# ashawkey/nerf2mesh

Measured on NVIDIA H100. Metric: ray-samples/sec (train step), higher is better.
Workload: dtype fp16

## Files before the change

nerf2mesh_b200/csrc/fused.cu:

```cuda
#include "n2m_common.cuh"
#include "s0_geom.cuh"
#include "mlp_common.cuh"
#include "../../include/n2m_b200_fused.h"

namespace n2m {
namespace {

__device__ __forceinline__ void bar_mlp() { asm volatile("bar.sync 1, 128;" ::: "memory"); }
__device__ __forceinline__ void sync_mlp() {
    wg::fence_async_smem();
    bar_mlp();
}
__device__ __forceinline__ void mbar_arrive1(uint64_t* bar) {
    asm volatile("mbarrier.arrive.shared::cta.b64 _, [%0];" :: "r"(wg::smem_u32(bar)) : "memory");
}

constexpr uint32_t kFwdThreads = 384;
constexpr uint32_t FF_W = 0, FF_A0 = FF_W + W_BYTES, FF_A1 = FF_A0 + kTileBytes, FF_H = FF_A1 + kTileBytes, FF_S1 = FF_H + kTileBytes,
                   FF_AS2 = FF_S1 + 8192, FF_BYTES = FF_AS2 + 4096;

__device__ __forceinline__ void bar_group(uint32_t g) {
    if (g == 0) asm volatile("bar.sync 2, 128;" ::: "memory");
    else asm volatile("bar.sync 3, 128;" ::: "memory");
}

__global__ void __launch_bounds__(kFwdThreads, 2)
k_s0_fwd_fused(n2m_s0_params p, const float4* __restrict__ recs, const int32_t* __restrict__ counters, const float* __restrict__ rays_o,
               const float* __restrict__ rays_d, const TableEntry* __restrict__ table, const int32_t* __restrict__ offsets,
               const uint8_t* __restrict__ wpack, uint8_t* __restrict__ enc_tiles, float4* __restrict__ out, float* __restrict__ spec_sq_sum) {
    extern __shared__ __align__(128) uint8_t smem[];
    __shared__ uint64_t bar_full[2], bar_empty[2];
    __shared__ float red[4];
    const uint32_t tid = threadIdx.x, warp = tid >> 5;
    const PartRange pr = part_range(counters, 0, 1);
    const uint32_t t1 = (pr.hi + kTile - 1) / kTile;
    if (pr.hi == 0 || blockIdx.x >= t1) return;
    const uint32_t my_tiles = (t1 - blockIdx.x + gridDim.x - 1) / gridDim.x;

    if (tid == 0) {
        wg::mbar_init(&bar_full[0], 1); wg::mbar_init(&bar_full[1], 1);
        wg::mbar_init(&bar_empty[0], 1); wg::mbar_init(&bar_empty[1], 1);
        wg::mbar_init_fence();
    }
    for (uint32_t i = tid; i < W_BYTES / 16; i += kFwdThreads)
        reinterpret_cast<uint4*>(smem + FF_W)[i] = __ldg(reinterpret_cast<const uint4*>(wpack) + i);
    if (tid < 128) *reinterpret_cast<uint4*>(smem + FF_AS2 + kChunk + tid * 16) = make_uint4(0, 0, 0, 0);
    wg::fence_async_smem();
    __syncthreads();

    if (warp >= 4) {
        const uint32_t g = (warp - 4) >> 2, r = tid - 128 - g * 128;
        uint8_t* buf = smem + (g ? FF_A1 : FF_A0);
        uint32_t k = 0;
        for (uint32_t it = g; it < my_tiles; it += 2, ++k) {
            const uint32_t tile = blockIdx.x + it * gridDim.x;
            float feat[kTileCols];
            encode_fwd_features<false>(p, recs, rays_o, rays_d, table, offsets, pr, tile * kTile + r, feat);
            if (r == 0) {
                asm volatile("cp.async.bulk.wait_group.read 0;" ::: "memory");
                wg::mbar_wait(&bar_empty[g], (k & 1) ^ 1);
            }
            bar_group(g);
            store_tile_row(buf, r, feat);
            wg::fence_async_smem();
            bar_group(g);
            if (r == 0) {
                asm volatile("cp.async.bulk.global.shared::cta.bulk_group [%0], [%1], %2;"
                             :: "l"(enc_tiles + (size_t)tile * kTileBytes), "r"(wg::smem_u32(buf)), "r"(kTileBytes) : "memory");
                asm volatile("cp.async.bulk.commit_group;" ::: "memory");
                mbar_arrive1(&bar_full[g]);
            }
        }
        if (r == 0) asm volatile("cp.async.bulk.wait_group 0;" ::: "memory");
    } else {
        float spec_sq = 0.f;
        const uint32_t r = sample_row(tid);
        for (uint32_t it = 0; it < my_tiles; ++it) {
            const uint32_t tile = blockIdx.x + it * gridDim.x, g = it & 1;
            const uint8_t* sA = smem + (g ? FF_A1 : FF_A0);
            wg::mbar_wait(&bar_full[g], (it >> 1) & 1);
            float sp[3];
            const float4 o = mlp_fwd_tile(sA, smem + FF_W, smem + FF_H, smem + FF_S1, smem + FF_S1, smem + FF_AS2, p.shading_full != 0,
                                          tid, sp, sync_mlp);
            const uint32_t j = tile * kTile + r;
            if (j < pr.hi) {
                out[j] = o;
                spec_sq += sp[0] * sp[0] + sp[1] * sp[1] + sp[2] * sp[2];
            }
            sync_mlp();
            if (tid == 0) mbar_arrive1(&bar_empty[g]);
        }
#pragma unroll
        for (int o = 16; o > 0; o >>= 1) spec_sq += __shfl_xor_sync(0xffffffffu, spec_sq, o);
        if ((tid & 31) == 0) red[warp] = spec_sq;
        bar_mlp();
        if (tid == 0 && spec_sq_sum) atomicAdd(spec_sq_sum, red[0] + red[1] + red[2] + red[3]);
// ... 29 lines not shown
```

nerf2mesh_b200/csrc/s0_geom.cuh:

```cuda
#pragma once
#include "n2m_common.cuh"
#include "../../include/n2m_b200_fused.h"

namespace n2m {
namespace {

constexpr uint32_t kTile = 128;
constexpr uint32_t kTileCols = 64;
constexpr uint32_t kTileBytes = kTile * kTileCols * 2;
constexpr uint32_t kChunkBytes = kTile * 16;
constexpr uint32_t kColXyz = 0, kColDens = 3, kColColor = 19, kColDir = 51;
constexpr uint32_t kLevels = 16;

struct __align__(8) TableEntry { float d; __half2 c; };

struct Sample {
    float x, y, z;
    float u, v, w;
    float dx, dy, dz;
};

__device__ __forceinline__ Sample sample_of(const float4 rec, const float* __restrict__ rays_o,
                                            const float* __restrict__ rays_d, const n2m_s0_params& p) {
    Sample s;
// ... 65 lines not shown
        zs[0] = z0 * mz;            zs[1] = zs[0] + mz;
    }
    const float wx[2] = {1 - fx, fx}, wy[2] = {1 - fy, fy}, wz[2] = {1 - fz, fz};
    const bool pow2 = (g.rows & (g.rows - 1)) == 0;
#pragma unroll
    for (int k = 0; k < 8; ++k) {
        const int ix = k & 1, iy = (k >> 1) & 1, iz = (k >> 2) & 1;
        const uint32_t raw = hashed ? (xs[ix] ^ ys[iy] ^ zs[iz]) : (xs[ix] + ys[iy] + zs[iz]);
        c.row[k] = wrap_row(raw, g.rows, pow2);
        c.w[k] = wx[ix] * wy[iy] * wz[iz];
    }
    if (left) {
        uint32_t lx, ly, lz;
        if (hashed) {
            lx = (x0 - 1u) ^ ys[0] ^ zs[0];
            ly = xs[0] ^ (ys[0] - 2654435761u) ^ zs[0];
            lz = xs[0] ^ ys[0] ^ (zs[0] - 805459861u);
        } else {
            lx = xs[0] - mx + ys[0] + zs[0];
            ly = xs[0] + ys[0] - my + zs[0];
            lz = xs[0] + ys[0] + zs[0] - mz;
        }
        left[0] = wrap_row(lx, g.rows, pow2);
        left[1] = wrap_row(ly, g.rows, pow2);
        left[2] = wrap_row(lz, g.rows, pow2);
    }
}

__device__ __forceinline__ uint32_t pack2(float a, float b) {
    const __half2 h = __floats2half2_rn(a, b);
    return *reinterpret_cast<const uint32_t*>(&h);
}

template <bool POINTS>
__device__ __forceinline__ bool
encode_fwd_features(const n2m_s0_params& p, const float4* __restrict__ recs, const float* __restrict__ rays_o,
                    const float* __restrict__ rays_d, const TableEntry* __restrict__ table, const int32_t* __restrict__ offsets,
                    const PartRange pr, uint32_t j, float (&feat)[kTileCols]) {
#pragma unroll
    for (uint32_t i = 0; i < kTileCols; ++i) feat[i] = 0.f;
    Sample s;
    const bool own = j >= pr.lo && j < pr.hi;
    bool active = own;
    if (own) {
        if (POINTS) {
            s.x = rays_o[3 * j]; s.y = rays_o[3 * j + 1]; s.z = rays_o[3 * j + 2];
            s.u = __fmul_rn(__fadd_rn(s.x, p.grid_bound), p.inv_2gb);
            s.v = __fmul_rn(__fadd_rn(s.y, p.grid_bound), p.inv_2gb);
            s.w = __fmul_rn(__fadd_rn(s.z, p.grid_bound), p.inv_2gb);
            s.dx = rays_d ? rays_d[3 * j] : 0.f; s.dy = rays_d ? rays_d[3 * j + 1] : 0.f; s.dz = rays_d ? rays_d[3 * j + 2] : 1.f;
        } else
        s = sample_of(recs[j], rays_o, rays_d, p);
        feat[kColXyz] = s.x; feat[kColXyz + 1] = s.y; feat[kColXyz + 2] = s.z;
        const float n2 = __fadd_rn(__fadd_rn(__fmul_rn(s.dx, s.dx), __fmul_rn(s.dy, s.dy)), __fmul_rn(s.dz, s.dz));
        const float nrm = __fsqrt_rn(fmaxf(n2, 1e-20f));
        feat[kColDir] = __fdiv_rn(s.dx, nrm); feat[kColDir + 1] = __fdiv_rn(s.dy, nrm); feat[kColDir + 2] = __fdiv_rn(s.dz, nrm);
        active = !((s.u < 0 || s.u > 1) || (s.v < 0 || s.v > 1) || (s.w < 0 || s.w > 1));
    } else {
        s.x = s.y = s.z = s.u = s.v = s.w = 0.5f; s.dx = s.dy = s.dz = 0.f;
    }
#pragma unroll
    for (uint32_t l = 0; l < kLevels; ++l) {
        const LevelGeom g = level_geom(offsets, l, p.S, p.base_res);
        Corners c; uint32_t base[3]; bool hashed;
        corners_of(g, s.u, s.v, s.w, c, base, hashed, nullptr);
        const TableEntry* tab = table + g.row0;
        if (active) {
            uint2 raw[8];
#pragma unroll
            for (int k = 0; k < 8; ++k) raw[k] = __ldg(reinterpret_cast<const uint2*>(tab + c.row[k]));
            float d = 0.f, c0 = 0.f, c1 = 0.f;
#pragma unroll
            for (int k = 0; k < 8; ++k) {
                const float2 cc = __half22float2(*reinterpret_cast<const __half2*>(&raw[k].y));
                d += c.w[k] * __uint_as_float(raw[k].x);
                c0 += c.w[k] * cc.x;
                c1 += c.w[k] * cc.y;
            }
            feat[kColDens + l] = d;
            feat[kColColor + 2 * l] = c0;
            feat[kColColor + 2 * l + 1] = c1;
        }
    }
    return own;
}

__device__ __forceinline__ float denc_col(const uint8_t* row, uint32_t col) {
    return __half2float(__ldg(reinterpret_cast<const __half*>(row + (col >> 3) * kChunkBytes + (col & 7) * 2)));
}

__device__ __forceinline__ void store_tile_row(uint8_t* img, uint32_t r, const float (&feat)[kTileCols]) {
    uint8_t* dst = img + r * 16;
#pragma unroll
    for (uint32_t ch = 0; ch < 8; ++ch) {
        uint4 q;
        q.x = pack2(feat[8 * ch + 0], feat[8 * ch + 1]);
        q.y = pack2(feat[8 * ch + 2], feat[8 * ch + 3]);
        q.z = pack2(feat[8 * ch + 4], feat[8 * ch + 5]);
        q.w = pack2(feat[8 * ch + 6], feat[8 * ch + 7]);
        *reinterpret_cast<uint4*>(dst + ch * kChunkBytes) = q;
    }
}

}
}
```

nerf2mesh_b200/csrc/stage0.cu:

```cuda
#include "march_core.cuh"
#include "s0_geom.cuh"
#include <cstdlib>
#include "../../include/n2m_b200_fused.h"

namespace n2m {
namespace {

using namespace march;

__global__ void __launch_bounds__(128)
k_s0_count(const float* __restrict__ rays_o, const float* __restrict__ rays_d, const float* __restrict__ aabb,
           const float* __restrict__ cam_nf, const uint8_t* __restrict__ bits, const float* __restrict__ noises,
           n2m_s0_params p, uint32_t N, int32_t* __restrict__ rays, float2* __restrict__ tbuf) {
    const uint32_t n = blockIdx.x * blockDim.x + threadIdx.x;
    if (n >= N) return;
    const MarchCfg c = make_cfg(p.bound, p.contract != 0, p.dt_gamma, p.max_steps, p.cascades, p.grid_size, bits);
    float near, far;
    near_far_aabb(rays_o + 3 * n, rays_d + 3 * n, aabb, p.min_near, near, far);
    if (cam_nf) {
        near = fmaxf(near, cam_nf[2 * n]);
        far = fminf(far, cam_nf[2 * n + 1]);
    }
    const float ox = rays_o[3 * n], oy = rays_o[3 * n + 1], oz = rays_o[3 * n + 2];
    const float dx = rays_d[3 * n], dy = rays_d[3 * n + 1], dz = rays_d[3 * n + 2];
// ... 134 lines not shown
        counters[3] = 0;
        counters[15] = 0;
        if (M > Mcap) counters[13] += 1;
        counters[14] = max(counters[14], (int32_t)M);
    }
    if (threadIdx.x <= kPartSlots) {
        const uint32_t e = threadIdx.x;
        const uint32_t first = part_first_ray(N, e);
        const uint32_t off = (e == kPartSlots || first >= N) ? M : (uint32_t)rays[2 * first];
        counters[4 + e] = (int32_t)min(min(off, M), Mcap);
    }
}

__global__ void __launch_bounds__(256)
k_s0_records(const int32_t* __restrict__ rays, const float2* __restrict__ tbuf, uint32_t N, uint32_t max_steps,
             uint32_t Mcap, float4* __restrict__ recs) {
    const uint32_t n = (blockIdx.x * blockDim.x + threadIdx.x) >> 5;
    const uint32_t lane = threadIdx.x & 31;
    if (n >= N) return;
    const uint32_t off = (uint32_t)rays[2 * n], cnt = (uint32_t)rays[2 * n + 1];
    const float2* slab = tbuf + (size_t)n * max_steps;
    for (uint32_t k = lane; k < cnt; k += 32) {
        const uint32_t j = off + k;
        if (j >= Mcap) break;
        const float2 td = slab[k];
        recs[j] = make_float4(td.x, td.y, td.x + td.y, __int_as_float((int)n));
    }
}

template <bool POINTS>
__device__ __forceinline__ void
encode_fwd_tile(const n2m_s0_params& p, const float4* __restrict__ recs,
                const float* __restrict__ rays_o, const float* __restrict__ rays_d,
                const TableEntry* __restrict__ table, const int32_t* __restrict__ offsets,
                uint8_t* __restrict__ enc_tiles, const PartRange pr, uint32_t nparts, uint32_t tile) {
    float feat[kTileCols];
    const bool own = encode_fwd_features<POINTS>(p, recs, rays_o, rays_d, table, offsets, pr, tile * kTile + threadIdx.x, feat);
    if (nparts > 1 && !own) return;
    store_tile_row(enc_tiles + (size_t)tile * kTileBytes, threadIdx.x, feat);
}

template <bool POINTS>
__global__ void __launch_bounds__(kTile, 6)
k_s0_encode_fwd(n2m_s0_params p, const float4* __restrict__ recs, const int32_t* __restrict__ counters,
                const float* __restrict__ rays_o, const float* __restrict__ rays_d,
                const TableEntry* __restrict__ table, const int32_t* __restrict__ offsets,
                uint8_t* __restrict__ enc_tiles, uint32_t part, uint32_t nparts) {
    const PartRange pr = part_range(counters, part, nparts);
    if (pr.hi <= pr.lo) return;
    const uint32_t t1 = (pr.hi + kTile - 1) / kTile;
#pragma unroll 1
    for (uint32_t tile = pr.lo / kTile + blockIdx.x; tile < t1; tile += gridDim.x)
        encode_fwd_tile<POINTS>(p, recs, rays_o, rays_d, table, offsets, enc_tiles, pr, nparts, tile);
}

__device__ __forceinline__ float tv_grad(const TableEntry* __restrict__ tab, const Corners& c, const uint32_t base[3],
                                         const uint32_t left[3], uint32_t res, float w) {
    const int right_corner[3] = {1, 2, 4};
    const float centre = __ldg(&tab[c.row[0]].d);
    float rv[3], lv[3];
#pragma unroll
    for (int d = 0; d < 3; ++d) {
        rv[d] = __ldg(&tab[c.row[right_corner[d]]].d);
        lv[d] = base[d] > 0 ? __ldg(&tab[left[d]].d) : 0.f;
    }
    float sum = 0.f, sq = 0.f;
#pragma unroll
    for (int d = 0; d < 3; ++d) {
        if (base[d] < res) { const float dv = centre - rv[d]; sum += dv; sq += dv * dv; }
        if (base[d] > 0) { const float dv = centre - lv[d]; sum += dv; sq += dv * dv; }
    }
    return w * sum * rsqrtf(sq + 1e-9f);
}

constexpr uint32_t kDenseGroupLevels = 5;
constexpr uint32_t kHashedGroupLevels = 1;
constexpr uint32_t kLevelGroups = 1 + (kLevels - kDenseGroupLevels + kHashedGroupLevels - 1) / kHashedGroupLevels;

__device__ __forceinline__ uint32_t group_first_level(uint32_t grp) {
    return grp == 0 ? 0u : min(kLevels, kDenseGroupLevels + (grp - 1) * kHashedGroupLevels);
}

__device__ __forceinline__ uint64_t l2_evict_last() {
    uint64_t pol;
    asm("createpolicy.fractional.L2::evict_last.b64 %0, 1.0;" : "=l"(pol));
    return pol;
}
__device__ __forceinline__ void red_add_v4(float4* dst, float a, float b, float c, uint64_t pol) {
    asm volatile("red.global.add.L2::cache_hint.v4.f32 [%0], {%1, %2, %3, %4}, %5;"
                 :: "l"(dst), "f"(a), "f"(b), "f"(c), "f"(0.f), "l"(pol) : "memory");
}

template <bool SCATTER, bool TV>
__device__ __forceinline__ void
encode_bwd_visit(const n2m_s0_params& p, const float4* __restrict__ recs,
                 const float* __restrict__ rays_o, const float* __restrict__ rays_d,
                 const uint8_t* __restrict__ denc_tiles, const TableEntry* __restrict__ table,
                 const int32_t* __restrict__ offsets, float4* __restrict__ gtable, float* __restrict__ loss_scale,
                 const PartRange pr, uint32_t tile, uint32_t l0, uint32_t l1, int32_t* tv_counts) {
    static_assert(SCATTER != TV, "a launch either scatters the feature gradients or evaluates TV");
    const uint32_t r = threadIdx.x;
    const uint32_t lane = r & 31;
    const uint32_t j = tile * kTile + r;
    Sample s;
    bool active = j >= pr.lo && j < pr.hi;
    if (active) {
        s = sample_of(recs[j], rays_o, rays_d, p);
        active = !((s.u < 0 || s.u > 1) || (s.v < 0 || s.v > 1) || (s.w < 0 || s.w > 1));
    } else {
        s.x = s.y = s.z = s.u = s.v = s.w = 0.5f; s.dx = s.dy = s.dz = 0.f;
    }

    const uint8_t* img = denc_tiles + (size_t)tile * kTileBytes + r * 16;
    bool bad = false;
    float tvw_lane = 0.f;
    if (TV) {
        const float mag = fmaxf(fabsf(s.x), fmaxf(fabsf(s.y), fabsf(s.z)));
        const bool outer = p.grid_bound > 1 && mag > 1;
        const float lam = outer ? p.lambda_tv * 10 : p.lambda_tv;
        tvw_lane = active ? lam / 6 * loss_scale[0] : 0.f;
        const bool mine = j >= pr.lo && j < pr.hi;
        const uint32_t m_out = __ballot_sync(0xffffffffu, mine && outer), m_in = __ballot_sync(0xffffffffu, mine && !outer);
        if (lane == 0 && l0 == 0) {
            if (m_in) atomicAdd(tv_counts + 3, (int)__popc(m_in));
            if (m_out) atomicAdd(tv_counts + 15, (int)__popc(m_out));
        }
    }
#pragma unroll 1
    for (uint32_t l = l0; l < l1; ++l) {
        const LevelGeom lg = level_geom(offsets, l, p.S, p.base_res);
        Corners c; uint32_t base[3]; bool hashed; uint32_t left[3];
        corners_of(lg, s.u, s.v, s.w, c, base, hashed, TV ? left : nullptr);
        float tvw = tvw_lane;
        float4* gt = gtable + lg.row0;
// ... 31 lines not shown
                }
            }
            const bool tail = lane == 31 || ((heads >> (lane + 1)) & 1u);
            issue = active && tail;
        }
        if (issue) {
            if (SCATTER) {
#pragma unroll
                const uint64_t pol = l2_evict_last();
#pragma unroll
                for (int k = 0; k < 8; ++k) red_add_v4(gt + c.row[k], vd[k], v0[k], v1[k], pol);
            }
            if (TV) atomicAdd(&gt[c.row[0]].x, tv_grad(table + lg.row0, c, base, left, lg.res, tvw));
        }
    }
    if (SCATTER && bad) loss_scale[3] = 1.f;
}

template <bool SCATTER, bool TV>
__global__ void __launch_bounds__(kTile)
k_s0_encode_bwd(n2m_s0_params p, const float4* __restrict__ recs, const int32_t* __restrict__ counters,
                const float* __restrict__ rays_o, const float* __restrict__ rays_d,
                const uint8_t* __restrict__ denc_tiles, const TableEntry* __restrict__ table,
                const int32_t* __restrict__ offsets, float4* __restrict__ gtable, float* __restrict__ loss_scale,
                uint32_t part, uint32_t nparts) {
    const PartRange pr = part_range(counters, part, nparts);
    if (pr.hi <= pr.lo) return;
    const uint32_t t0 = pr.lo / kTile, nt = (pr.hi + kTile - 1) / kTile - t0;
#pragma unroll 1
    for (uint32_t item = blockIdx.x; item < kLevelGroups * nt; item += gridDim.x) {
        const uint32_t grp = item / nt;
        encode_bwd_visit<SCATTER, TV>(p, recs, rays_o, rays_d, denc_tiles, table, offsets, gtable, loss_scale, pr, t0 + item % nt,
                                      group_first_level(grp), group_first_level(grp + 1), const_cast<int32_t*>(counters));
    }
}

__host__ __device__ __forceinline__ uint32_t mix32(uint32_t h) {
    h ^= h >> 16; h *= 0x85ebca6bu; h ^= h >> 13; h *= 0xc2b2ae35u; h ^= h >> 16;
    return h;
}
__host__ __device__ __forceinline__ float tv_random_coord(uint32_t seed, uint32_t idx, uint32_t axis) {
    return (float)(mix32(mix32(idx * 3u + axis) ^ (seed * 0x9e3779b9u)) >> 8) * (1.0f / 16777216.0f);
}

__global__ void __launch_bounds__(128)
k_s0_tv_random(n2m_s0_params p, const int32_t* __restrict__ counters, const TableEntry* __restrict__ table,
               const int32_t* __restrict__ offsets, float4* __restrict__ gtable, const float* __restrict__ loss_scale, uint32_t B,
               float* __restrict__ dump) {
    float lam = 0.f;
    if (p.grid_bound > 1) {
        if (counters[3] == 0) lam += p.lambda_tv;
        if (counters[15] == 0) lam += p.lambda_tv * 10;
    } else if (counters[3] + counters[15] == 0) lam = p.lambda_tv;
    if (dump) lam = p.lambda_tv;
    if (!(lam > 0.f)) return;
    const uint32_t i = blockIdx.x * blockDim.x + threadIdx.x;
    if (i >= B) return;
    const uint32_t seed = (uint32_t)loss_scale[2];
    const float u = tv_random_coord(seed, i, 0), v = tv_random_coord(seed, i, 1), w = tv_random_coord(seed, i, 2);
    if (dump) { dump[3 * i] = u; dump[3 * i + 1] = v; dump[3 * i + 2] = w; }
    const float tvw = lam / 6 * loss_scale[0];
#pragma unroll 1
    for (uint32_t l = 0; l < kLevels; ++l) {
        const LevelGeom lg = level_geom(offsets, l, p.S, p.base_res);
        Corners c; uint32_t base[3]; bool hashed; uint32_t left[3];
        corners_of(lg, u, v, w, c, base, hashed, left);
// ... 211 lines not shown
    cmaster[i] = c;
}

__global__ void __launch_bounds__(256)
k_s0_unpack_tables(const TableEntry* __restrict__ table, const float2* __restrict__ cmaster, uint32_t rows,
                   float* __restrict__ ed, float* __restrict__ ec) {
    const uint32_t i = blockIdx.x * blockDim.x + threadIdx.x;
    if (i >= rows) return;
    ed[i] = table[i].d;
    ec[2 * i] = cmaster[i].x; ec[2 * i + 1] = cmaster[i].y;
}

__global__ void __launch_bounds__(256)
k_s0_unpack_grads(const float4* __restrict__ gtable, uint32_t rows, const float* __restrict__ loss_scale,
                  float* __restrict__ gd, float* __restrict__ gc) {
    const uint32_t i = blockIdx.x * blockDim.x + threadIdx.x;
    if (i >= rows) return;
    const float inv = 1.0f / loss_scale[0];
    const float4 g = gtable[i];
    gd[i] = g.x * inv; gc[2 * i] = g.y * inv; gc[2 * i + 1] = g.z * inv;
}

}
}

using namespace n2m;

static bool g_serial_march = false;

static inline uint32_t part_grid(uint32_t Mcap, uint32_t nparts) {
    return nparts <= 1 ? Mcap / kTile : div_up(Mcap / kTile, nparts) + 1;
}

template <bool SCATTER, bool TV>
static uint32_t encode_bwd_grid(uint32_t Mcap, uint32_t nparts, uint32_t share = 1) {
    static int per_sm = 0;
    if (!per_sm) {
        cudaOccupancyMaxActiveBlocksPerMultiprocessor(&per_sm, k_s0_encode_bwd<SCATTER, TV>, kTile, 0);
        if (per_sm <= 0) per_sm = 1;
    }
    return min(max(1u, (uint32_t)(per_sm * num_sms()) / (nparts * share)), kLevelGroups * part_grid(Mcap, nparts));
}

constexpr uint32_t kTvDeviceShare = 2;

extern "C" {

int n2m_s0_set_serial_march(int on) { g_serial_march = on != 0; return 0; }
int n2m_s0_pack_tables(const float* emb_density, const float* emb_color, uint32_t rows, void* table, void* color_master,
                       n2m_stream_t stream) {
    N2M_REQUIRE(emb_density && emb_color && table && color_master, "s0_pack_tables", "null pointer");
    k_s0_pack_tables<<<div_up(rows, 256u), 256, 0, as_stream(stream)>>>(emb_density, emb_color, rows,
                                                                         static_cast<TableEntry*>(table), static_cast<float2*>(color_master));
    return check_launch("s0_pack_tables");
}

int n2m_s0_unpack_tables(const void* table, const void* color_master, uint32_t rows, float* emb_density, float* emb_color,
                         n2m_stream_t stream) {
    N2M_REQUIRE(emb_density && emb_color && table && color_master, "s0_unpack_tables", "null pointer");
    k_s0_unpack_tables<<<div_up(rows, 256u), 256, 0, as_stream(stream)>>>(static_cast<const TableEntry*>(table),
                                                                           static_cast<const float2*>(color_master), rows, emb_density, emb_color);
    return check_launch("s0_unpack_tables");
}

int n2m_s0_unpack_grads(const void* gtable, uint32_t rows, const float* loss_scale, float* g_density, float* g_color,
                        n2m_stream_t stream) {
    N2M_REQUIRE(gtable && loss_scale && g_density && g_color, "s0_unpack_grads", "null pointer");
    k_s0_unpack_grads<<<div_up(rows, 256u), 256, 0, as_stream(stream)>>>(static_cast<const float4*>(gtable), rows, loss_scale, g_density, g_color);
    return check_launch("s0_unpack_grads");
}

int n2m_s0_march(const n2m_s0_params* p, const float* rays_o, const float* rays_d, const float* aabb,
                 const float* cam_near_far, const uint8_t* bitfield, const float* noises, uint32_t N, int32_t* rays,
                 int32_t* counters, float* tbuf, void* recs, uint32_t Mcap, n2m_stream_t stream) {
    N2M_REQUIRE(p && rays && counters, "s0_march", "null pointer");
    cudaStream_t st = as_stream(stream);
    if (N == 0) { cudaMemsetAsync(counters, 0, 4 * sizeof(int32_t), st); return 0; }
    N2M_REQUIRE(rays_o && rays_d && aabb && bitfield && noises && tbuf && recs, "s0_march", "null pointer");
    N2M_REQUIRE(p->max_steps > 0 && p->grid_size > 0 && p->cascades > 0, "s0_march", "bad params");
    if (g_serial_march)
        k_s0_count<<<div_up(N, 128u), 128, 0, st>>>(rays_o, rays_d, aabb, cam_near_far, bitfield, noises, *p, N, rays,
// ... 48 lines not shown
    return check_launch("s0_grid_update");
}

int n2m_s0_packbits_dev(const float* grid, uint32_t nbytes, const float* mean_density, float density_thresh, uint8_t* bitfield,
                        n2m_stream_t stream) {
    N2M_REQUIRE(grid && mean_density && bitfield, "s0_packbits_dev", "null pointer");
    if (nbytes == 0) return 0;
    k_s0_packbits_dev<<<div_up(nbytes, 256u), 256, 0, as_stream(stream)>>>(grid, nbytes, mean_density, density_thresh, bitfield);
    return check_launch("s0_packbits_dev");
}

int n2m_s0_gen_rays(const float* poses, uint32_t num_poses, const float* intrinsics_host, uint32_t H, uint32_t W,
                    const int32_t* img_idx, const int32_t* pix_idx, const uint8_t* images, uint32_t C, uint32_t N,
                    float* rays_o, float* rays_d, float* gt, n2m_stream_t stream) {
    if (N == 0) return 0;
    N2M_REQUIRE(poses && intrinsics_host && img_idx && pix_idx && rays_o && rays_d, "s0_gen_rays", "null pointer");
    N2M_REQUIRE(num_poses > 0 && H > 0 && W > 0, "s0_gen_rays", "empty pose set or image");
    N2M_REQUIRE(!gt || (images && (C == 3 || C == 4)), "s0_gen_rays", "gt requested without images, or channels not 3 / 4");
    k_s0_gen_rays<<<div_up(N, 256u), 256, 0, as_stream(stream)>>>(poses, intrinsics_host[0], intrinsics_host[1], intrinsics_host[2],
                                                                 intrinsics_host[3], W, img_idx, pix_idx, images, H * W, C, N,
                                                                 rays_o, rays_d, gt);
    return check_launch("s0_gen_rays");
}

int n2m_s0_encode_bwd(const n2m_s0_params* p, const void* recs, const int32_t* counters, uint32_t Mcap,
                      const float* rays_o, const float* rays_d, const void* denc_tiles, const void* table,
                      const int32_t* offsets, void* gtable, const float* loss_scale, uint32_t part, uint32_t nparts,
                      n2m_stream_t stream) {
    N2M_REQUIRE(p && recs && counters && rays_o && rays_d && denc_tiles && table && offsets && gtable && loss_scale,
                "s0_encode_bwd", "null pointer");
    N2M_REQUIRE(p->num_levels == kLevels, "s0_encode_bwd", "fused path supports num_levels == 16");
    N2M_REQUIRE(Mcap % kTile == 0 && Mcap > 0, "s0_encode_bwd", "Mcap must be a positive multiple of 128");
    N2M_REQUIRE(valid_parts(part, nparts), "s0_encode_bwd", "nparts must be 1, 2, 4 or 8 and part < nparts");
    k_s0_encode_bwd<true, false><<<encode_bwd_grid<true, false>(Mcap, nparts), kTile, 0, as_stream(stream)>>>(
        *p, static_cast<const float4*>(recs), counters, rays_o, rays_d, static_cast<const uint8_t*>(denc_tiles),
        static_cast<const TableEntry*>(table), offsets, static_cast<float4*>(gtable), const_cast<float*>(loss_scale), part, nparts);
    return check_launch("s0_encode_bwd");
}

int n2m_s0_tv(const n2m_s0_params* p, const void* recs, const int32_t* counters, uint32_t Mcap, const float* rays_o,
              const float* rays_d, const void* table, const int32_t* offsets, void* gtable, const float* loss_scale,
              n2m_stream_t stream) {
    N2M_REQUIRE(p && recs && counters && rays_o && rays_d && table && offsets && gtable && loss_scale, "s0_tv", "null pointer");
    N2M_REQUIRE(Mcap % kTile == 0 && Mcap > 0, "s0_tv", "Mcap must be a positive multiple of 128");
    if (!(p->lambda_tv > 0)) return 0;
    k_s0_encode_bwd<false, true><<<encode_bwd_grid<false, true>(Mcap, 1, kTvDeviceShare), kTile, 0, as_stream(stream)>>>(
        *p, static_cast<const float4*>(recs), counters, rays_o, rays_d, nullptr, static_cast<const TableEntry*>(table), offsets,
        static_cast<float4*>(gtable), const_cast<float*>(loss_scale), 0, 1);
    return check_launch("s0_tv");
}

int n2m_s0_tv_random(const n2m_s0_params* p, const int32_t* counters, const void* table, const int32_t* offsets, void* gtable,
                     const float* loss_scale, uint32_t num_points, float* dump, n2m_stream_t stream) {
    N2M_REQUIRE(p && counters && table && offsets && gtable && loss_scale, "s0_tv_random", "null pointer");
    if (!(p->lambda_tv > 0) || num_points == 0) return 0;
    k_s0_tv_random<<<div_up(num_points, 128u), 128, 0, as_stream(stream)>>>(*p, counters, static_cast<const TableEntry*>(table), offsets,
                                                                            static_cast<float4*>(gtable), loss_scale, num_points, dump);
    return check_launch("s0_tv_random");
}

int n2m_s0_composite_loss(const n2m_s0_params* p, const void* out, const void* recs, const int32_t* rays,
                          const int32_t* counters, uint32_t N, uint32_t Mcap, const float* gt, const float* bg,
                          const float* loss_scale, void* dout, float* image, float* weights_sum, float* depth,
                          float* loss_out, uint32_t part, uint32_t nparts, n2m_stream_t stream) {
    (void)Mcap;
    if (N == 0) return 0;
    N2M_REQUIRE(p && out && recs && rays && counters && gt && bg && loss_scale && dout && image && weights_sum && depth && loss_out,
                "s0_composite_loss", "null pointer");
    N2M_REQUIRE(valid_parts(part, nparts), "s0_composite_loss", "nparts must be 1, 2, 4 or 8 and part < nparts");
// ... 10 lines not shown
```

include/n2m_b200_fused.h:

```cpp
#ifndef N2M_B200_FUSED_H
#define N2M_B200_FUSED_H

#include "n2m_b200.h"

#ifdef __cplusplus
extern "C" {
#endif

typedef struct {
    float bound;
    float grid_bound;
    float inv_2gb;
    float dt_gamma;
    float min_near;
    float T_thresh;
    float S;
    float lambda_mask;
    float lambda_specular;
    float lambda_tv;
    float lambda_entropy;
    uint32_t contract;
    uint32_t max_steps;
    uint32_t cascades;
    uint32_t grid_size;
    uint32_t num_levels;
    uint32_t base_res;
    uint32_t shading_full;
    uint32_t gt_has_alpha;
} n2m_s0_params;

int n2m_s0_init(void);

int n2m_s0_set_serial_march(int on);

int n2m_s0_tv(const n2m_s0_params* p, const void* recs, const int32_t* counters, uint32_t Mcap, const float* rays_o,
              const float* rays_d, const void* table, const int32_t* offsets, void* gtable, const float* loss_scale,
              n2m_stream_t stream);
int n2m_s0_tv_random(const n2m_s0_params* p, const int32_t* counters, const void* table, const int32_t* offsets, void* gtable,
                     const float* loss_scale, uint32_t num_points, float* dump, n2m_stream_t stream);

uint32_t n2m_s0_wpack_bytes(void);
uint32_t n2m_s0_mlp_param_count(void);

int n2m_s0_pack_weights(const float* mlp_params, void* wpack, n2m_stream_t stream);

int n2m_s0_pack_tables(const float* emb_density, const float* emb_color, uint32_t rows,
                       void* table, void* color_master, n2m_stream_t stream);
int n2m_s0_unpack_tables(const void* table, const void* color_master, uint32_t rows,
                         float* emb_density, float* emb_color, n2m_stream_t stream);
int n2m_s0_unpack_grads(const void* gtable, uint32_t rows, const float* loss_scale,
                        float* g_density, float* g_color, n2m_stream_t stream);

int n2m_s0_march(const n2m_s0_params* p, const float* rays_o, const float* rays_d, const float* aabb,
                 const float* cam_near_far, const uint8_t* bitfield, const float* noises, uint32_t N,
                 int32_t* rays, int32_t* counters, float* tbuf, void* recs, uint32_t Mcap,
                 n2m_stream_t stream);

int n2m_s0_encode_fwd(const n2m_s0_params* p, const void* recs, const int32_t* counters, uint32_t Mcap,
                      const float* rays_o, const float* rays_d, const void* table, const int32_t* offsets,
                      void* enc_tiles, uint32_t part, uint32_t nparts, n2m_stream_t stream);

int n2m_s0_encode_points(const n2m_s0_params* p, const float* xyz, const float* dirs, const int32_t* counters, uint32_t Pcap,
                         const void* table, const int32_t* offsets, void* enc_tiles, n2m_stream_t stream);

int n2m_s0_grid_points(uint32_t H, uint32_t first_cell, uint32_t count, float cas_bound, const float* noise, float* xyz,
                       n2m_stream_t stream);
// ... 79 lines not shown
```

nerf2mesh_b200/stage0.py:

```python
import ctypes
import math
from ctypes import c_float, c_uint32

import numpy as np
import torch

from . import _lib
from ._lib import F, I, P, U, call, ptr, stream
from .gridencoder.grid import level_offsets


class S0Params(ctypes.Structure):
    _fields_ = [(n, c_float) for n in ("bound", "grid_bound", "inv_2gb", "dt_gamma", "min_near", "T_thresh", "S",
                                       "lambda_mask", "lambda_specular", "lambda_tv", "lambda_entropy")] + \
               [(n, c_uint32) for n in ("contract", "max_steps", "cascades", "grid_size", "num_levels", "base_res",
                                        "shading_full", "gt_has_alpha")]


PP = ctypes.POINTER(S0Params)

_lib.register({
    "n2m_s0_init": [],
    "n2m_s0_set_serial_march": [I],
    "n2m_s0_tv": [PP, P, P, U, P, P, P, P, P, P, P],
    "n2m_s0_tv_random": [PP, P, P, P, P, P, U, P, P],
    "n2m_s0_pack_weights": [P, P, P],
    "n2m_s0_pack_tables": [P, P, U, P, P, P],
    "n2m_s0_unpack_tables": [P, P, U, P, P, P],
    "n2m_s0_unpack_grads": [P, U, P, P, P, P],
    "n2m_s0_march": [PP, P, P, P, P, P, P, U, P, P, P, P, U, P],
    "n2m_s0_encode_fwd": [PP, P, P, U, P, P, P, P, P, U, U, P],
    "n2m_s0_encode_points": [PP, P, P, P, U, P, P, P, P],
    "n2m_s0_grid_points": [U, U, U, F, P, P, P],
    "n2m_s0_grid_update": [P, U, F, P, P],
    "n2m_s0_packbits_dev": [P, U, P, F, P, P],
    "n2m_s0_mlp_fwd": [PP, P, P, U, P, P, P, U, U, P],
    "n2m_s0_composite_loss": [PP, P, P, P, P, U, U, P, P, P, P, P, P, P, P, U, U, P],
    "n2m_s0_mlp_bwd": [PP, P, P, P, U, P, P, P, P, U, U, P],
    "n2m_s0_encode_bwd": [PP, P, P, U, P, P, P, P, P, P, P, U, U, P],
    "n2m_s0_adam_head": [P, P, P],
    "n2m_s0_adam_tables": [P, P, P, P, P, U, P, F, P],
    "n2m_s0_adam_tables_keep": [P, P, P, P, P, U, P, F, P],
    "n2m_s0_adam_mlp": [P, P, P, P, P, P, F, P],
    "n2m_s0_adam_post": [P, P],
    "n2m_mark_untrained_grid": [P, U, P, U, P, F, P, F, U, U, P, P, P],
    "n2m_s0_fwd_fused": [PP, P, P, U, P, P, P, P, P, P, P, P, P],
    "n2m_s0_render_begin": [PP, P, P, P, P, U, P, P, P, P, P, P, P, P],
    "n2m_s0_render_rounds": [PP, P, P, P, U, P, U, P, P, P, P, P, P, P, U, P, P, P, P, P, P, P],
    "n2m_s0_render_finish": [P, P, P, F, U, P],
    "n2m_s0_ema_update": [P, P, P, P, P, P, U, F, P],
    "n2m_s0_ema_swap": [P, P, P, P, P, P, U, P, P],
})
_lib.lib.n2m_s0_wpack_bytes.restype = c_uint32
_lib.lib.n2m_s0_mlp_param_count.restype = c_uint32

MLP_LAYOUT = [
# ... 742 lines not shown
```

Before: 275.3 million.

## Precompute level descriptors in shared memory and prefetch next level's hash-grid corners

Per-level grid geometry (scale, strides, hashing and wrap mode) is now computed once per block into shared memory instead of being rederived from offsets for every sample and level. The encoder loop is software-pipelined so the eight corner loads for level l+1 are issued before level l is interpolated, and features are packed straight into fp16 words instead of a 64-float array. Out-of-range samples return early. The TV device share constant is also changed from 2 to 3. The aim is to hide gather latency and reduce register and ALU pressure, at the cost of more live registers for the prefetched corners.

```diff
diff --git a/nerf2mesh_b200/csrc/fused.cu b/nerf2mesh_b200/csrc/fused.cu
--- a/nerf2mesh_b200/csrc/fused.cu
+++ b/nerf2mesh_b200/csrc/fused.cu
@@ -31,6 +31,7 @@
     extern __shared__ __align__(128) uint8_t smem[];
     __shared__ uint64_t bar_full[2], bar_empty[2];
     __shared__ float red[4];
+    __shared__ LevelDesc geo[kLevels];
     const uint32_t tid = threadIdx.x, warp = tid >> 5;
     const PartRange pr = part_range(counters, 0, 1);
     const uint32_t t1 = (pr.hi + kTile - 1) / kTile;
@@ -46,7 +47,7 @@
         reinterpret_cast<uint4*>(smem + FF_W)[i] = __ldg(reinterpret_cast<const uint4*>(wpack) + i);
     if (tid < 128) *reinterpret_cast<uint4*>(smem + FF_AS2 + kChunk + tid * 16) = make_uint4(0, 0, 0, 0);
     wg::fence_async_smem();
-    __syncthreads();
+    load_level_descs(geo, offsets, p);
 
     if (warp >= 4) {
         const uint32_t g = (warp - 4) >> 2, r = tid - 128 - g * 128;
@@ -54,14 +55,14 @@
         uint32_t k = 0;
         for (uint32_t it = g; it < my_tiles; it += 2, ++k) {
             const uint32_t tile = blockIdx.x + it * gridDim.x;
-            float feat[kTileCols];
-            encode_fwd_features<false>(p, recs, rays_o, rays_d, table, offsets, pr, tile * kTile + r, feat);
+            uint32_t row[kTileCols / 2];
+            encode_fwd_features<false>(p, recs, rays_o, rays_d, table, geo, pr, tile * kTile + r, row);
             if (r == 0) {
                 asm volatile("cp.async.bulk.wait_group.read 0;" ::: "memory");
                 wg::mbar_wait(&bar_empty[g], (k & 1) ^ 1);
             }
             bar_group(g);
-            store_tile_row(buf, r, feat);
+            store_tile_row(buf, r, row);
             wg::fence_async_smem();
             bar_group(g);
             if (r == 0) {
diff --git a/nerf2mesh_b200/csrc/s0_geom.cuh b/nerf2mesh_b200/csrc/s0_geom.cuh
--- a/nerf2mesh_b200/csrc/s0_geom.cuh
+++ b/nerf2mesh_b200/csrc/s0_geom.cuh
@@ -121,75 +121,135 @@
     return *reinterpret_cast<const uint32_t*>(&h);
 }
 
+enum : uint32_t { kWrapNone = 0, kWrapMask = 1, kWrapMod = 2 };
+
+struct __align__(16) LevelDesc {
+    float scale;
+    uint32_t row0, rows, wrap;
+    uint32_t mx, my, mz;
+    uint32_t hashed;
+};
+
+__device__ __forceinline__ void load_level_descs(LevelDesc (&geo)[kLevels], const int32_t* __restrict__ offsets, const n2m_s0_params& p) {
+    if (threadIdx.x < kLevels) {
+        const LevelGeom g = level_geom(offsets, threadIdx.x, p.S, p.base_res);
+        LevelDesc d;
+        d.scale = g.scale; d.row0 = g.row0; d.rows = g.rows;
+        const uint32_t s1 = g.res + 1;
+        uint32_t stride = 1;
+        d.mx = d.my = d.mz = 0;
+        if (stride <= g.rows) { d.mx = stride; stride *= s1; }
+        if (stride <= g.rows) { d.my = stride; stride *= s1; }
+        if (stride <= g.rows) { d.mz = stride; stride *= s1; }
+        d.hashed = stride > g.rows;
+        d.wrap = !d.hashed ? kWrapNone : (g.rows & (g.rows - 1)) == 0 ? kWrapMask : kWrapMod;
+        geo[threadIdx.x] = d;
+    }
+    __syncthreads();
+}
+
+__device__ __forceinline__ void desc_corners(const LevelDesc& g, float u, float v, float w, Corners& c) {
+    const float pu = u * g.scale + 0.5f, pv = v * g.scale + 0.5f, pw = w * g.scale + 0.5f;
+    const float fu0 = floorf(pu), fv0 = floorf(pv), fw0 = floorf(pw);
+    const uint32_t x0 = fu0, y0 = fv0, z0 = fw0;
+    const float fx = pu - (float)x0, fy = pv - (float)y0, fz = pw - (float)z0;
+    const float wx[2] = {1 - fx, fx}, wy[2] = {1 - fy, fy}, wz[2] = {1 - fz, fz};
+#pragma unroll
+    for (int k = 0; k < 8; ++k) c.w[k] = wx[k & 1] * wy[(k >> 1) & 1] * wz[(k >> 2) & 1];
+    uint32_t xs[2], ys[2], zs[2];
+    if (g.hashed) {
+        xs[0] = x0;                 xs[1] = x0 + 1u;
+        ys[0] = y0 * 2654435761u;   ys[1] = ys[0] + 2654435761u;
+        zs[0] = z0 * 805459861u;    zs[1] = zs[0] + 805459861u;
+#pragma unroll
+        for (int k = 0; k < 8; ++k) c.row[k] = xs[k & 1] ^ ys[(k >> 1) & 1] ^ zs[(k >> 2) & 1];
+    } else {
+        xs[0] = x0 * g.mx;          xs[1] = xs[0] + g.mx;
+        ys[0] = y0 * g.my;          ys[1] = ys[0] + g.my;
+        zs[0] = z0 * g.mz;          zs[1] = zs[0] + g.mz;
+#pragma unroll
+        for (int k = 0; k < 8; ++k) c.row[k] = xs[k & 1] + ys[(k >> 1) & 1] + zs[(k >> 2) & 1];
+    }
+    if (g.wrap == kWrapMask) {
+#pragma unroll
+        for (int k = 0; k < 8; ++k) c.row[k] &= g.rows - 1;
+    } else if (g.wrap == kWrapMod) {
+#pragma unroll
+        for (int k = 0; k < 8; ++k) c.row[k] %= g.rows;
+    }
+}
+
+__device__ __forceinline__ void put_col(uint32_t (&row)[kTileCols / 2], uint32_t col, float v) {
+    row[col >> 1] |= (uint32_t)__half_as_ushort(__float2half_rn(v)) << (16 * (col & 1));
+}
+
+__device__ __forceinline__ void load_corners(const TableEntry* __restrict__ tab, const Corners& c, uint2 (&raw)[8]) {
+#pragma unroll
+    for (int k = 0; k < 8; ++k) raw[k] = __ldg(reinterpret_cast<const uint2*>(tab + c.row[k]));
+}
+
 template <bool POINTS>
 __device__ __forceinline__ bool
 encode_fwd_features(const n2m_s0_params& p, const float4* __restrict__ recs, const float* __restrict__ rays_o,
-                    const float* __restrict__ rays_d, const TableEntry* __restrict__ table, const int32_t* __restrict__ offsets,
-                    const PartRange pr, uint32_t j, float (&feat)[kTileCols]) {
-#pragma unroll
-    for (uint32_t i = 0; i < kTileCols; ++i) feat[i] = 0.f;
+                    const float* __restrict__ rays_d, const TableEntry* __restrict__ table, const LevelDesc (&geo)[kLevels],
+                    const PartRange pr, uint32_t j, uint32_t (&row)[kTileCols / 2]) {
+#pragma unroll
+    for (uint32_t i = 0; i < kTileCols / 2; ++i) row[i] = 0u;
+    const bool own = j >= pr.lo && j < pr.hi;
+    if (!own) return false;
     Sample s;
-    const bool own = j >= pr.lo && j < pr.hi;
-    bool active = own;
-    if (own) {
-        if (POINTS) {
-            s.x = rays_o[3 * j]; s.y = rays_o[3 * j + 1]; s.z = rays_o[3 * j + 2];
-            s.u = __fmul_rn(__fadd_rn(s.x, p.grid_bound), p.inv_2gb);
-            s.v = __fmul_rn(__fadd_rn(s.y, p.grid_bound), p.inv_2gb);
-            s.w = __fmul_rn(__fadd_rn(s.z, p.grid_bound), p.inv_2gb);
-            s.dx = rays_d ? rays_d[3 * j] : 0.f; s.dy = rays_d ? rays_d[3 * j + 1] : 0.f; s.dz = rays_d ? rays_d[3 * j + 2] : 1.f;
-        } else
-        s = sample_of(recs[j], rays_o, rays_d, p);
-        feat[kColXyz] = s.x; feat[kColXyz + 1] = s.y; feat[kColXyz + 2] = s.z;
-        const float n2 = __fadd_rn(__fadd_rn(__fmul_rn(s.dx, s.dx), __fmul_rn(s.dy, s.dy)), __fmul_rn(s.dz, s.dz));
-        const float nrm = __fsqrt_rn(fmaxf(n2, 1e-20f));
-        feat[kColDir] = __fdiv_rn(s.dx, nrm); feat[kColDir + 1] = __fdiv_rn(s.dy, nrm); feat[kColDir + 2] = __fdiv_rn(s.dz, nrm);
-        active = !((s.u < 0 || s.u > 1) || (s.v < 0 || s.v > 1) || (s.w < 0 || s.w > 1));
-    } else {
-        s.x = s.y = s.z = s.u = s.v = s.w = 0.5f; s.dx = s.dy = s.dz = 0.f;
-    }
+    if (POINTS) {
+        s.x = rays_o[3 * j]; s.y = rays_o[3 * j + 1]; s.z = rays_o[3 * j + 2];
+        s.u = __fmul_rn(__fadd_rn(s.x, p.grid_bound), p.inv_2gb);
+        s.v = __fmul_rn(__fadd_rn(s.y, p.grid_bound), p.inv_2gb);
+        s.w = __fmul_rn(__fadd_rn(s.z, p.grid_bound), p.inv_2gb);
+        s.dx = rays_d ? rays_d[3 * j] : 0.f; s.dy = rays_d ? rays_d[3 * j + 1] : 0.f; s.dz = rays_d ? rays_d[3 * j + 2] : 1.f;
+    } else
+    s = sample_of(recs[j], rays_o, rays_d, p);
+    put_col(row, kColXyz, s.x); put_col(row, kColXyz + 1, s.y); put_col(row, kColXyz + 2, s.z);
+    const float n2 = __fadd_rn(__fadd_rn(__fmul_rn(s.dx, s.dx), __fmul_rn(s.dy, s.dy)), __fmul_rn(s.dz, s.dz));
+    const float nrm = __fsqrt_rn(fmaxf(n2, 1e-20f));
+    put_col(row, kColDir, __fdiv_rn(s.dx, nrm)); put_col(row, kColDir + 1, __fdiv_rn(s.dy, nrm));
+    put_col(row, kColDir + 2, __fdiv_rn(s.dz, nrm));
+    if ((s.u < 0 || s.u > 1) || (s.v < 0 || s.v > 1) || (s.w < 0 || s.w > 1)) return true;
+    Corners c;
+    uint2 raw[8];
+    desc_corners(geo[0], s.u, s.v, s.w, c);
+    load_corners(table + geo[0].row0, c, raw);
 #pragma unroll
     for (uint32_t l = 0; l < kLevels; ++l) {
-        const LevelGeom g = level_geom(offsets, l, p.S, p.base_res);
-        Corners c; uint32_t base[3]; bool hashed;
-        corners_of(g, s.u, s.v, s.w, c, base, hashed, nullptr);
-        const TableEntry* tab = table + g.row0;
-        if (active) {
-            uint2 raw[8];
-#pragma unroll
-            for (int k = 0; k < 8; ++k) raw[k] = __ldg(reinterpret_cast<const uint2*>(tab + c.row[k]));
-            float d = 0.f, c0 = 0.f, c1 = 0.f;
-#pragma unroll
-            for (int k = 0; k < 8; ++k) {
-                const float2 cc = __half22float2(*reinterpret_cast<const __half2*>(&raw[k].y));
-                d += c.w[k] * __uint_as_float(raw[k].x);
-                c0 += c.w[k] * cc.x;
-                c1 += c.w[k] * cc.y;
-            }
-            feat[kColDens + l] = d;
-            feat[kColColor + 2 * l] = c0;
-            feat[kColColor + 2 * l + 1] = c1;
+        float w[8]; uint2 cur[8];
+#pragma unroll
+        for (int k = 0; k < 8; ++k) { w[k] = c.w[k]; cur[k] = raw[k]; }
+        if (l + 1 < kLevels) {
+            desc_corners(geo[l + 1], s.u, s.v, s.w, c);
+            load_corners(table + geo[l + 1].row0, c, raw);
         }
-    }
-    return own;
+        float d = 0.f, c0 = 0.f, c1 = 0.f;
+#pragma unroll
+        for (int k = 0; k < 8; ++k) {
+            const float2 cc = __half22float2(*reinterpret_cast<const __half2*>(&cur[k].y));
+            d += w[k] * __uint_as_float(cur[k].x);
+            c0 += w[k] * cc.x;
+            c1 += w[k] * cc.y;
+        }
+        put_col(row, kColDens + l, d);
+        put_col(row, kColColor + 2 * l, c0);
+        put_col(row, kColColor + 2 * l + 1, c1);
+    }
+    return true;
 }
 
 __device__ __forceinline__ float denc_col(const uint8_t* row, uint32_t col) {
     return __half2float(__ldg(reinterpret_cast<const __half*>(row + (col >> 3) * kChunkBytes + (col & 7) * 2)));
 }
 
-__device__ __forceinline__ void store_tile_row(uint8_t* img, uint32_t r, const float (&feat)[kTileCols]) {
+__device__ __forceinline__ void store_tile_row(uint8_t* img, uint32_t r, const uint32_t (&row)[kTileCols / 2]) {
     uint8_t* dst = img + r * 16;
 #pragma unroll
-    for (uint32_t ch = 0; ch < 8; ++ch) {
-        uint4 q;
-        q.x = pack2(feat[8 * ch + 0], feat[8 * ch + 1]);
-        q.y = pack2(feat[8 * ch + 2], feat[8 * ch + 3]);
-        q.z = pack2(feat[8 * ch + 4], feat[8 * ch + 5]);
-        q.w = pack2(feat[8 * ch + 6], feat[8 * ch + 7]);
-        *reinterpret_cast<uint4*>(dst + ch * kChunkBytes) = q;
-    }
-}
-
-}
-}
+    for (uint32_t ch = 0; ch < 8; ++ch)
+        *reinterpret_cast<uint4*>(dst + ch * kChunkBytes) = make_uint4(row[4 * ch], row[4 * ch + 1], row[4 * ch + 2], row[4 * ch + 3]);
+}
+
+}
+}
diff --git a/nerf2mesh_b200/csrc/stage0.cu b/nerf2mesh_b200/csrc/stage0.cu
--- a/nerf2mesh_b200/csrc/stage0.cu
+++ b/nerf2mesh_b200/csrc/stage0.cu
@@ -190,12 +190,12 @@
 __device__ __forceinline__ void
 encode_fwd_tile(const n2m_s0_params& p, const float4* __restrict__ recs,
                 const float* __restrict__ rays_o, const float* __restrict__ rays_d,
-                const TableEntry* __restrict__ table, const int32_t* __restrict__ offsets,
+                const TableEntry* __restrict__ table, const LevelDesc (&geo)[kLevels],
                 uint8_t* __restrict__ enc_tiles, const PartRange pr, uint32_t nparts, uint32_t tile) {
-    float feat[kTileCols];
-    const bool own = encode_fwd_features<POINTS>(p, recs, rays_o, rays_d, table, offsets, pr, tile * kTile + threadIdx.x, feat);
+    uint32_t row[kTileCols / 2];
+    const bool own = encode_fwd_features<POINTS>(p, recs, rays_o, rays_d, table, geo, pr, tile * kTile + threadIdx.x, row);
     if (nparts > 1 && !own) return;
-    store_tile_row(enc_tiles + (size_t)tile * kTileBytes, threadIdx.x, feat);
+    store_tile_row(enc_tiles + (size_t)tile * kTileBytes, threadIdx.x, row);
 }
 
 template <bool POINTS>
@@ -204,12 +204,15 @@
                 const float* __restrict__ rays_o, const float* __restrict__ rays_d,
                 const TableEntry* __restrict__ table, const int32_t* __restrict__ offsets,
                 uint8_t* __restrict__ enc_tiles, uint32_t part, uint32_t nparts) {
+    __shared__ LevelDesc geo[kLevels];
     const PartRange pr = part_range(counters, part, nparts);
     if (pr.hi <= pr.lo) return;
     const uint32_t t1 = (pr.hi + kTile - 1) / kTile;
+    if (pr.lo / kTile + blockIdx.x >= t1) return;
+    load_level_descs(geo, offsets, p);
 #pragma unroll 1
     for (uint32_t tile = pr.lo / kTile + blockIdx.x; tile < t1; tile += gridDim.x)
-        encode_fwd_tile<POINTS>(p, recs, rays_o, rays_d, table, offsets, enc_tiles, pr, nparts, tile);
+        encode_fwd_tile<POINTS>(p, recs, rays_o, rays_d, table, geo, enc_tiles, pr, nparts, tile);
 }
 
 __device__ __forceinline__ float tv_grad(const TableEntry* __restrict__ tab, const Corners& c, const uint32_t base[3],
@@ -642,7 +645,7 @@
     return min(max(1u, (uint32_t)(per_sm * num_sms()) / (nparts * share)), kLevelGroups * part_grid(Mcap, nparts));
 }
 
-constexpr uint32_t kTvDeviceShare = 2;
+constexpr uint32_t kTvDeviceShare = 3;
 
 extern "C" {
 
```

New measurement: 273.1 million, median of 6. Within noise of the previous version (-0.8%).

## Use whole-SM 1024-thread scatter walker kernel for partitioned encode backward

Applied to the files above, without the earlier changes.

Adds a scatter-only backward kernel that packs eight 128-sample tile walkers into each 1024-thread block, capped at 56 registers, with a grid of at most one block per SM per partition. It is used by default when the backward pass is split into more than one partition. The aim is to let each partition's scatter sit on a fixed share of SMs so it overlaps better with the other partition's MLP backward, instead of flooding the device with small blocks. A runtime switch selects the form. The register cap may cause spills, and the smaller grid may reduce parallelism. A profiling timeline script is also added.

```diff
diff --git a/include/n2m_b200_fused.h b/include/n2m_b200_fused.h
--- a/include/n2m_b200_fused.h
+++ b/include/n2m_b200_fused.h
@@ -32,6 +32,8 @@
 int n2m_s0_init(void);
 
 int n2m_s0_set_serial_march(int on);
+
+int n2m_s0_set_scatter_form(int form);
 
 int n2m_s0_tv(const n2m_s0_params* p, const void* recs, const int32_t* counters, uint32_t Mcap, const float* rays_o,
               const float* rays_d, const void* table, const int32_t* offsets, void* gtable, const float* loss_scale,
diff --git a/nerf2mesh_b200/csrc/stage0.cu b/nerf2mesh_b200/csrc/stage0.cu
--- a/nerf2mesh_b200/csrc/stage0.cu
+++ b/nerf2mesh_b200/csrc/stage0.cu
@@ -257,7 +257,7 @@
                  const int32_t* __restrict__ offsets, float4* __restrict__ gtable, float* __restrict__ loss_scale,
                  const PartRange pr, uint32_t tile, uint32_t l0, uint32_t l1, int32_t* tv_counts) {
     static_assert(SCATTER != TV, "a launch either scatters the feature gradients or evaluates TV");
-    const uint32_t r = threadIdx.x;
+    const uint32_t r = threadIdx.x & (kTile - 1);
     const uint32_t lane = r & 31;
     const uint32_t j = tile * kTile + r;
     Sample s;
@@ -355,6 +355,25 @@
         const uint32_t grp = item / nt;
         encode_bwd_visit<SCATTER, TV>(p, recs, rays_o, rays_d, denc_tiles, table, offsets, gtable, loss_scale, pr, t0 + item % nt,
                                       group_first_level(grp), group_first_level(grp + 1), const_cast<int32_t*>(counters));
+    }
+}
+
+constexpr uint32_t kWholeSmThreads = 1024;
+
+__global__ void __maxnreg__(56)
+k_s0_scatter_walkers(n2m_s0_params p, const float4* __restrict__ recs, const int32_t* __restrict__ counters,
+                     const float* __restrict__ rays_o, const float* __restrict__ rays_d, const uint8_t* __restrict__ denc_tiles,
+                     const int32_t* __restrict__ offsets, float4* __restrict__ gtable, float* __restrict__ loss_scale,
+                     uint32_t part, uint32_t nparts) {
+    const PartRange pr = part_range(counters, part, nparts);
+    if (pr.hi <= pr.lo) return;
+    const uint32_t t0 = pr.lo / kTile, nt = (pr.hi + kTile - 1) / kTile - t0;
+#pragma unroll 1
+    for (uint32_t item = blockIdx.x * (kWholeSmThreads / kTile) + threadIdx.x / kTile; item < kLevelGroups * nt;
+         item += gridDim.x * (kWholeSmThreads / kTile)) {
+        const uint32_t grp = item / nt;
+        encode_bwd_visit<true, false>(p, recs, rays_o, rays_d, denc_tiles, nullptr, offsets, gtable, loss_scale, pr, t0 + item % nt,
+                                      group_first_level(grp), group_first_level(grp + 1), nullptr);
     }
 }
 
@@ -632,6 +651,8 @@
     return nparts <= 1 ? Mcap / kTile : div_up(Mcap / kTile, nparts) + 1;
 }
 
+static int g_scatter_form = 0;
+
 template <bool SCATTER, bool TV>
 static uint32_t encode_bwd_grid(uint32_t Mcap, uint32_t nparts, uint32_t share = 1) {
     static int per_sm = 0;
@@ -642,11 +663,20 @@
     return min(max(1u, (uint32_t)(per_sm * num_sms()) / (nparts * share)), kLevelGroups * part_grid(Mcap, nparts));
 }
 
+static uint32_t scatter_walkers_grid(uint32_t Mcap, uint32_t nparts) {
+    return min(max(1u, (uint32_t)num_sms() / nparts), div_up(kLevelGroups * part_grid(Mcap, nparts), kWholeSmThreads / kTile));
+}
+
 constexpr uint32_t kTvDeviceShare = 2;
 
 extern "C" {
 
 int n2m_s0_set_serial_march(int on) { g_serial_march = on != 0; return 0; }
+int n2m_s0_set_scatter_form(int form) {
+    N2M_REQUIRE(form >= 0 && form <= 2, "s0_set_scatter_form", "form must be 0, 1 or 2");
+    g_scatter_form = form;
+    return 0;
+}
 int n2m_s0_pack_tables(const float* emb_density, const float* emb_color, uint32_t rows, void* table, void* color_master,
                        n2m_stream_t stream) {
     N2M_REQUIRE(emb_density && emb_color && table && color_master, "s0_pack_tables", "null pointer");
@@ -761,9 +791,15 @@
     N2M_REQUIRE(p->num_levels == kLevels, "s0_encode_bwd", "fused path supports num_levels == 16");
     N2M_REQUIRE(Mcap % kTile == 0 && Mcap > 0, "s0_encode_bwd", "Mcap must be a positive multiple of 128");
     N2M_REQUIRE(valid_parts(part, nparts), "s0_encode_bwd", "nparts must be 1, 2, 4 or 8 and part < nparts");
-    k_s0_encode_bwd<true, false><<<encode_bwd_grid<true, false>(Mcap, nparts), kTile, 0, as_stream(stream)>>>(
-        *p, static_cast<const float4*>(recs), counters, rays_o, rays_d, static_cast<const uint8_t*>(denc_tiles),
-        static_cast<const TableEntry*>(table), offsets, static_cast<float4*>(gtable), const_cast<float*>(loss_scale), part, nparts);
+    const bool whole_sm = g_scatter_form ? g_scatter_form == 2 : nparts > 1;
+    if (whole_sm)
+        k_s0_scatter_walkers<<<scatter_walkers_grid(Mcap, nparts), kWholeSmThreads, 0, as_stream(stream)>>>(
+            *p, static_cast<const float4*>(recs), counters, rays_o, rays_d, static_cast<const uint8_t*>(denc_tiles), offsets,
+            static_cast<float4*>(gtable), const_cast<float*>(loss_scale), part, nparts);
+    else
+        k_s0_encode_bwd<true, false><<<encode_bwd_grid<true, false>(Mcap, nparts), kTile, 0, as_stream(stream)>>>(
+            *p, static_cast<const float4*>(recs), counters, rays_o, rays_d, static_cast<const uint8_t*>(denc_tiles),
+            static_cast<const TableEntry*>(table), offsets, static_cast<float4*>(gtable), const_cast<float*>(loss_scale), part, nparts);
     return check_launch("s0_encode_bwd");
 }
 
diff --git a/nerf2mesh_b200/stage0.py b/nerf2mesh_b200/stage0.py
--- a/nerf2mesh_b200/stage0.py
+++ b/nerf2mesh_b200/stage0.py
@@ -22,6 +22,7 @@
 _lib.register({
     "n2m_s0_init": [],
     "n2m_s0_set_serial_march": [I],
+    "n2m_s0_set_scatter_form": [I],
     "n2m_s0_tv": [PP, P, P, U, P, P, P, P, P, P, P],
     "n2m_s0_tv_random": [PP, P, P, P, P, P, U, P, P],
     "n2m_s0_pack_weights": [P, P, P],
diff --git a/profiles/step_timeline.py b/profiles/step_timeline.py
--- /dev/null
+++ b/profiles/step_timeline.py
@@ -0,0 +1,152 @@
+import argparse
+import json
+import os
+import re
+import subprocess
+import sys
+import tempfile
+
+import torch
+
+ROOT = os.path.dirname(os.path.dirname(os.path.abspath(__file__)))
+sys.path.insert(0, ROOT)
+
+CHAIN = ["k_s0_encode_fwd<false>", "k_mlp_fwd", "k_s0_composite_loss", "k_mlp_bwd", "scatter"]
+SCATTERS = ("k_s0_encode_bwd<true, false>", "k_s0_scatter_walkers")
+TV = "k_s0_encode_bwd<false, true>"
+
+
+def stage(name):
+    return "scatter" if name in SCATTERS else name
+
+
+def power_limit():
+    try:
+        r = subprocess.run(["nvidia-smi", "--query-gpu=power.limit", "--format=csv,noheader", "-i", "0"], capture_output=True,
+                           text=True, timeout=20)
+        return r.stdout.strip() or None
+    except Exception:
+        return None
+
+
+def short_name(name):
+    name = re.sub(r"^void ", "", name)
+    depth, cut = 0, len(name)
+    for i, ch in enumerate(name):
+        if ch == "<":
+            depth += 1
+        elif ch == ">":
+            depth -= 1
+        elif ch == "(" and depth == 0 and not name.startswith("(anonymous", i):
+            cut = i
+            break
+    return re.sub(r"^(?:\w+::|\(anonymous namespace\)::)+", "", name[:cut])
+
+
+def kernels_of(trace_path):
+    with open(trace_path) as f:
+        ks = [e for e in json.load(f)["traceEvents"] if e.get("cat") == "kernel"]
+    t0 = min(e["ts"] for e in ks)
+    out = [{"name": short_name(e["name"]), "stream": e["args"].get("stream"), "start_us": round(e["ts"] - t0, 2),
+            "end_us": round(e["ts"] + e["dur"] - t0, 2), "grid": e["args"].get("grid"), "block": e["args"].get("block")} for e in ks]
+    return sorted(out, key=lambda k: k["start_us"])
+
+
+def waits(ks):
+    by_stream = {}
+    for k in ks:
+        if stage(k["name"]) in CHAIN:
+            by_stream.setdefault(k["stream"], []).append(k)
+    parts = sorted((v for v in by_stream.values() if [stage(k["name"]) for k in v] == CHAIN), key=lambda c: c[0]["start_us"])
+    assert len(parts) == 2, {s: [k["name"] for k in v] for s, v in by_stream.items()}
+    comp, bwd, sc = 2, 3, 4
+    tv_end = max((k["end_us"] for k in ks if k["name"] == TV), default=None)
+
+    def gap(a, b):
+        return round(b["start_us"] - a["end_us"], 2)
+    return {
+        "part0_mlp_bwd": {"composite_end_us": parts[0][comp]["end_us"], "start_us": parts[0][bwd]["start_us"],
+                          "gap_us": gap(parts[0][comp], parts[0][bwd]), "tv_end_us": tv_end},
+        "part1_mlp_bwd": {"composite_end_us": parts[1][comp]["end_us"], "start_us": parts[1][bwd]["start_us"],
+                          "gap_us": gap(parts[1][comp], parts[1][bwd]), "part0_mlp_bwd_end_us": parts[0][bwd]["end_us"],
+                          "part0_scatter_end_us": parts[0][sc]["end_us"]},
+        "part0_scatter": {"mlp_bwd_end_us": parts[0][bwd]["end_us"], "start_us": parts[0][sc]["start_us"],
+                          "gap_us": gap(parts[0][bwd], parts[0][sc]), "part1_mlp_bwd_end_us": parts[1][bwd]["end_us"]},
+        "scatters_end_us": max(p[sc]["end_us"] for p in parts),
+        "step_span_us": max(k["end_us"] for k in ks),
+    }
+
+
+def run(workload, warmup, trace_dir):
+    import bench
+    from torch.profiler import ProfilerActivity, profile
+    tr = bench.make_trainer(workload)
+    tr.nparts = 2
+    assert tr.cfg.lambda_tv > 0
+    n_batches = 8
+    host, grid, bits = bench.make_batches(n_batches, 1000, True, workload)
+    dev = [{k: v.cuda(non_blocking=True) for k, v in b.items()} for b in host]
+    tr.set_occupancy(bits, grid)
+
+    def tup(b):
+        return (b["ro"], b["rd"], b["gt"], b["bg"], b["noises"]) + ((b["cnf"],) if "cnf" in b else ())
+
+    it = [0]
+
+    def one_step(use_graph):
+        b = dev[it[0] % n_batches]
+        tr.step(b["ro"], b["rd"], b["gt"], b["bg"], b["noises"], shading="full", use_graph=use_graph,
+                next_batch=tup(dev[(it[0] + 1) % n_batches]), cam_near_far=b.get("cnf"))
+        it[0] += 1
+
+    for i in range(warmup):
+        one_step(use_graph=i % 4 < 2)
+    torch.cuda.synchronize()
+    out = {"workload": workload, "device": torch.cuda.get_device_properties(0).name, "power_limit": power_limit(),
+           "nparts": tr.nparts, "lambda_tv": tr.cfg.lambda_tv}
+    for mode in ("eager", "graph"):
+        path = os.path.join(trace_dir, f"step_timeline_{workload}_{mode}.pt.trace.json")
+        with profile(activities=[ProfilerActivity.CUDA]) as prof:
+            one_step(use_graph=mode == "graph")
+            torch.cuda.synchronize()
+        prof.export_chrome_trace(path)
+        ks = kernels_of(path)
+        out[mode] = {"waits": waits(ks), "kernels": ks}
+    return out
+
+
+def report(r):
+    print(f"== {r['workload']}  {r['device']}  power limit {r['power_limit']}")
+    for mode in ("eager", "graph"):
+        print(f"-- {mode} step: kernel, stream, start_us, end_us, grid x block")
+        for k in r[mode]["kernels"]:
+            print(f"   {k['name'][:40]:<40} {str(k['stream']):>4} {k['start_us']:>9.2f} {k['end_us']:>9.2f}  {k['grid']} x {k['block']}")
+        w = r[mode]["waits"]
+        a, b, c = w["part0_mlp_bwd"], w["part1_mlp_bwd"], w["part0_scatter"]
+        print(f"   part 0 k_mlp_bwd: composite ends {a['composite_end_us']:.2f}, starts {a['start_us']:.2f} (gap {a['gap_us']:.2f} us); "
+              f"TV ends {a['tv_end_us']}")
+        print(f"   part 1 k_mlp_bwd: composite ends {b['composite_end_us']:.2f}, starts {b['start_us']:.2f} (gap {b['gap_us']:.2f} us); "
+              f"part 0's k_mlp_bwd ends {b['part0_mlp_bwd_end_us']:.2f}, part 0's scatter ends {b['part0_scatter_end_us']:.2f}")
+        print(f"   part 0 scatter:   its k_mlp_bwd ends {c['mlp_bwd_end_us']:.2f}, starts {c['start_us']:.2f} (gap {c['gap_us']:.2f} us); "
+              f"part 1's k_mlp_bwd ends {c['part1_mlp_bwd_end_us']:.2f}")
+    print(json.dumps({k: ({"waits": v["waits"]} if k in ("eager", "graph") else v) for k, v in r.items()}), flush=True)
+
+
+def main():
+    ap = argparse.ArgumentParser()
+    ap.add_argument("--warmup", type=int, default=10)
+    ap.add_argument("--workload", nargs="+", default=["lego_stage0_converged", "garden_stage0"])
+    ap.add_argument("--trace-dir", default=None, help="keep the Chrome traces here (default: a temporary directory)")
+    args = ap.parse_args()
+    if not torch.cuda.is_available():
+        raise SystemExit("step_timeline.py: no CUDA device")
+    torch.cuda.set_device(0)
+    with tempfile.TemporaryDirectory() as tmp:
+        trace_dir = args.trace_dir or tmp
+        os.makedirs(trace_dir, exist_ok=True)
+        for w in args.workload:
+            report(run(w, args.warmup, trace_dir))
+
+
+if __name__ == "__main__":
+    main()
```

After: 274.6 million before, 286.6 million after, median of 6. 4.4% higher.
